# Fahien/rayca

Hardware: AMD Instinct MI355X
Metric: Mrays/sec (primary+shadow), 1920x1080 Sponza 1spp (higher is better)
Workload: dtype f32; 1 GPU; sponza-STAND-IN procedural atrium 271,568 tris, 1920x1080, primary + 1 shadow ray (Pathtracer max_depth=1, NEE, 1 point light), 1 spp; width=1920, height=1080, triangles=271568, bvh_nodes=135379, bvh_built_on=gpu (bvh_build.hip; same tree as the host builder), rays_per_frame=4146938, frames_in_flight=4, tiling=rows in bands of 8 dealt over 1 rank(s), frame_gather=none, launched_by=single process

## Files before the change

### __graft_entry__.py

```python
from __future__ import annotations

import os
import subprocess
import sys

ROOT = os.path.dirname(os.path.abspath(__file__))
CSRC = os.path.join(ROOT, "rayca_amd", "csrc")
LIB = os.path.join(CSRC, "librayca_hip.so")
HIPCC = os.environ.get("HIPCC", "/opt/rocm/bin/hipcc")
VARIANT_FLAGS = ["-DRAYCA_GEN_WAVES_PER_BLOCK=4", "-DRAYCA_COLD_ARGS=0"]
VARIANT_LIB = os.path.join(CSRC, "variants", "librayca_gen_earlier.so")

COMMON = ["-O3", "-std=c++17", "-fPIC", "-ffp-contract=off", "-fno-fast-math", "-Wall", "-Wno-unused-function",
          "-Wno-unused-result"]


def _stale(target, sources):
    if not os.path.exists(target):
        return True
    t = os.path.getmtime(target)
    return any(os.path.getmtime(s) > t for s in sources)


def build(force: bool = False) -> None:
    srcs = [os.path.join(CSRC, f) for f in ("kernels.hip", "refill.hip", "refill.hpp", "flavour.hpp", "trace_core.inc", "bvh_build.hip", "api.inc", "select.inc", "scene.inc", "multi.inc", "post.inc", "aux_kernels.inc", "general.inc", "wavefront.inc", "surface.inc", "image_pass.inc", "denoise.inc", "denoise_variance.inc", "temporal.inc", "upsample.inc", "tonemap.inc",
                                            "host_scene.cpp", "host_scene.hpp", "device_types.hpp", "no_pk.hpp", "rayca_math.hpp", "staging.hpp", "libm_exact.hpp")]
    srcs.append(os.path.join(ROOT, "include", "rayca_hip.h"))
    if force or _stale(LIB, srcs) or _stale(VARIANT_LIB, srcs):
        host_obj = os.path.join(CSRC, "host_scene.o")
        jobs = [subprocess.Popen(["g++", *COMMON, "-c", os.path.join(CSRC, "host_scene.cpp"), "-o", host_obj, "-pthread"])]
        objs = []
        for unit in ("kernels", "refill", "bvh_build"):
            obj = os.path.join(CSRC, unit + ".o")
            objs.append(obj)
            jobs.append(subprocess.Popen([HIPCC, "--offload-arch=gfx950", *COMMON, "-c", os.path.join(CSRC, unit + ".hip"), "-o", obj]))
        os.makedirs(os.path.dirname(VARIANT_LIB), exist_ok=True)
        variant_obj = os.path.join(os.path.dirname(VARIANT_LIB), "kernels_gen_earlier.o")
        jobs.append(subprocess.Popen([HIPCC, "--offload-arch=gfx950", *COMMON, *VARIANT_FLAGS, "-c", os.path.join(CSRC, "kernels.hip"), "-o", variant_obj]))
        failed = [j.args for j in jobs if j.wait() != 0]
        if failed:
            raise subprocess.CalledProcessError(1, failed[0])
        subprocess.run([HIPCC, "--offload-arch=gfx950", "-shared", "-fPIC", *objs, host_obj, "-o", LIB, "-lpthread"], check=True)
        subprocess.run([HIPCC, "--offload-arch=gfx950", "-shared", "-fPIC", variant_obj, *objs[1:], host_obj, "-o", VARIANT_LIB, "-lpthread"], check=True)
    subprocess.run(["make", "-s", "-C", os.path.join(ROOT, "oracle")], check=True)
    build_cpp_host()
    build_cpp_host("resident_draw")
    build_microbench()
    if ROOT not in sys.path:
        sys.path.insert(0, ROOT)
    import rayca_amd
    from rayca_amd import abi, lib
    l = lib.load()
    for sym in abi.PRODUCT_SYMBOLS:
        getattr(l, sym)


def build_microbench() -> None:
    out_dir = os.path.join(ROOT, "tests", "microbench", "_build")
    os.makedirs(out_dir, exist_ok=True)
    for name, extra, deps in (("peaks", [], []), ("libm_compare", ["-ffp-contract=off", "-fno-fast-math"], [os.path.join(CSRC, "libm_exact.hpp")])):
        src, exe = os.path.join(ROOT, "tests", "microbench", name + ".hip"), os.path.join(out_dir, name)
        if _stale(exe, [src] + deps):
            subprocess.run([HIPCC, "--offload-arch=gfx950", "-O3", "-std=c++17", *extra, src, "-o", exe], check=True)
# ... 55 lines not shown
```

### rayca_amd/csrc/api.inc

```
#include <dlfcn.h>

#include <algorithm>
#include <atomic>
#include <chrono>
#include <condition_variable>
#include <functional>
#include <memory>
#include <cstdio>
#include <cstdlib>
#include <cstring>
#include <mutex>
#include <string>
#include <thread>
#include <vector>

#include "refill.hpp"
#include "staging.hpp"

using namespace rayca;

namespace {

thread_local std::string g_last_error;

// ... 564 lines not shown
  return timed_launch(f.log, f.stream, refill ? RAYCA_KERNEL_SHADOW_REFILL : RAYCA_KERNEL_WF_SHADOW, f.timing, true, [&] {
    if (refill)
      launch_shadow_refill(gen0, sph, stats, lgrid, sp.lds_bytes, f.stream, *f.dscene, f.fp, q.in, q.in_count, sa, g, c->heads_b, c->counters, tl);
    else
      hipLaunchKernelGGL(kh, dim3(lgrid), dim3(kBlock), sp.lds_bytes, f.stream, *f.dscene, f.fp, q.in, q.in_count, wb, f.pb, g, c->counters, tl);
    return RAYCA_OK;
  });
}

GenChoice choose_generation(Frame& f, uint32_t g) {
  RaycaScene* s = f.s;
  const LaunchPlan& plan = f.plan;
  RaycaScene::Tune& tu = s->tune[plan.mode == kModePath ? 1 : 0][g == 0 ? 0 : 1];
  GenChoice ch{f.all_formats ? format_forced() : 0, false, false, false};
  const int refill_env = knobs().refill;
  const bool refill_possible = f.fused && plan.mode == kModeFlat && plan.ordered && s->dev.ref_leaf_of != nullptr;
  const int refill_forced = !refill_possible ? 0 : (f.opts.camera_rays == RAYCA_CAMERA_REFILL ? 1 : (f.opts.camera_rays == RAYCA_CAMERA_GENERATION ? 0 : refill_env));
  ch.refill = refill_forced > 0;
  bool kernel_pending = false;
  if (refill_possible && f.all_formats && refill_forced < 0) {
    std::lock_guard<std::mutex> tune_lock(s->tune_mu);
    if (tu.refill >= 0) ch.refill = tu.refill != 0;
    else if (f.pb.npix >= 65536u && !plan.stats && tu.refill_launched < 8u) {
      ch.refill = (tu.refill_launched++ & 1u) != 0;
      ch.refill_cal = true;
      if (ch.format < 0) ch.format = 1;
    } else {
      kernel_pending = true;
    }
  }
  const bool can_tune = plan.ordered && s->dev.ref_leaf_of != nullptr && wide_forced() < 0 && f.all_formats;
  if (can_tune && !ch.refill_cal && !kernel_pending) {
    const int cls = g == 0 ? 0 : 1;
    if (f.frame_format[cls] == -2) {
      std::lock_guard<std::mutex> tune_lock(s->tune_mu);
      f.frame_format[cls] = -1;
      if (tu.decided >= 0) f.frame_format[cls] = tu.decided;
      else if (f.pb.npix >= 65536u && !plan.stats && tu.launched < 16u) {
        f.frame_format[cls] = (int)(tu.launched++ & 3u);
        f.frame_calibrates[cls] = true;
      }
    }
    if (f.frame_format[cls] >= 0) ch.format = f.frame_format[cls];
    ch.calibrating = f.frame_calibrates[cls];
  }
  return ch;
}

int32_t fused_generation(Frame& f, uint32_t g, const GenQueues& q) {
  RaycaScene* s = f.s;
  FrameCtx* c = f.c;
  const GenChoice ch = choose_generation(f, g);
  const bool park = RAYCA_PARK_CTX && f.plan.mode == kModePath;
  const TravPlan tp = plan_traversal(s, f.plan.ordered, g, ch.format, park ? path_lds_entries() : kMaxLdsEntries);
  f.node_format |= (traits(tp.trav).wide ? (g == 0 ? 1u : 2u) : 0u) | (traits(tp.trav).half ? (g == 0 ? 4u : 8u) : 0u) | (ch.calibrating ? 256u : 0u) |
                   (ch.refill_cal ? 512u : 0u) | (ch.refill ? 1024u : 0u);
  const StackPlan sp = tp.stack;
  const uint32_t block = ch.refill ? (uint32_t)kBlock : (uint32_t)kGenBlock;
  const size_t lds_bytes = ((size_t)sp.lds_entries * 4u + (park ? (size_t)kCtxQuads * 16u : 0u)) * block;
  const bool sph = s->host.sphere_count != 0;
  GenKernel k = pick_kernel(f.plan.mode, g == 0, f.fused, tp.trav, sph, f.plan.stats);
  const RefillFlavour rf{tp.trav, sph, f.plan.stats};
  const uint32_t batches = g == 0 ? f.fp.tile_count : (f.pb.npix + 63u) / 64u;
  const uint32_t grid_mult = knobs().grid_mult;
  uint32_t grid = 0;
  TraceLaunch tl{};
  int32_t rc = persistent_grid(s, ch.refill ? flat_refill_kernel(rf) : reinterpret_cast<const void*>(k), lds_bytes, batches, true, f.in_flight, grid_mult, grid, block / 64u);
  if (rc != RAYCA_OK || (rc = bind_stack(c, sp, grid, tl, block)) != RAYCA_OK) return rc;
  const uint32_t ticket_forced = knobs().ticket;
  tl.ticket = ticket_forced ? ticket_forced : ticket_policy(batches, grid, block / 64u);
  size_t ev = 0;
  rc = timed_launch(f.log, f.stream, ch.refill ? RAYCA_KERNEL_FLAT_REFILL : RAYCA_KERNEL_GENERATION, f.timing || ch.calibrating || ch.refill_cal, true, [&] {
    if (ch.refill)
      launch_flat_refill(rf, grid, lds_bytes, f.stream, *f.dscene, f.fp, c->heads, f.rgba8, f.rgba32f, c->counters, tl);
    else
      hipLaunchKernelGGL(k, dim3(grid), dim3(kGenBlock), lds_bytes, f.stream,
                         GenArgs{*f.dscene, f.fp, c->heads, q.in, q.in_count, q.out, q.out_count, f.pb, g, f.rgba8, f.rgba32f, c->counters, tl});
    return RAYCA_OK;
  }, &ev);
  if (rc != RAYCA_OK) return rc;
  if (ch.calibrating) f.tune_events.push_back({g == 0 ? 0 : 1, ev, ch.format, -1});
  if (ch.refill_cal) f.tune_events.push_back({0, ev, ch.format, ch.refill ? 1 : 0});
  return RAYCA_OK;
}

int32_t stack_machine(Frame& f) {
  RaycaScene* s = f.s;
  FrameCtx* c = f.c;
  const RaycaConfig& cfg = f.cfg;
  GeneralKernel k = pick_general_kernel(s->dev.ref_leaf_of != nullptr, s->host.sphere_count != 0, f.plan.stats);
  const StackPlan sp = plan_stack(s->host.max_depth);
  uint32_t grid = 0;
  int32_t rc = persistent_grid(s, reinterpret_cast<const void*>(k), sp.lds_bytes, f.fp.tile_count, false, 1u, 0u, grid);
  if (rc != RAYCA_OK) return rc;
  uint32_t levels = 1;
  if (cfg.integrator == RAYCA_INTEGRATOR_PATHTRACER) levels = cfg.russian_roulette ? 64u : (cfg.max_depth ? cfg.max_depth : 1u);
  else if (cfg.integrator == RAYCA_INTEGRATOR_RAYTRACER || cfg.integrator == RAYCA_INTEGRATOR_SCRATCHER) levels = cfg.max_depth + 2u;
  if (levels > 256u) return fail(RAYCA_ERR_UNSUPPORTED, "max_depth too large for the path-vertex stack");
  GFrameStore store{};
  store.threads = grid * kBlock;
  store.levels = levels + 1u;
  if ((rc = grow_behind_pass(c, c->frames, (size_t)store.levels * 8u * store.threads * 16u)) != RAYCA_OK) return rc;
  store.frames = static_cast<float4*>(c->frames.ptr);
  if (cfg.direct_sampler == RAYCA_SAMPLER_MIS) {
    if ((rc = grow_behind_pass(c, c->mis_samples, (size_t)2u * kMisMaxSamples * store.threads * 16u)) != RAYCA_OK) return rc;
    store.samples = static_cast<float4*>(c->mis_samples.ptr);
  }
  TraceLaunch tl{};
  if ((rc = bind_stack(c, sp, grid, tl)) != RAYCA_OK) return rc;
  tl.ticket = f.fp.tile_count >= 16u * grid ? 2u : 1u;
  c->heads_clean = false;
  return timed_launch(f.log, f.stream, RAYCA_KERNEL_OTHER, f.timing, true, [&]() -> int32_t {
    HIP_TRY(hipMemsetAsync(c->heads, 0, 8 * kHeadStride * sizeof(uint32_t), f.stream));
// ... 771 lines not shown
```

### rayca_amd/csrc/kernels.hip

```cpp
#include "no_pk.hpp"
RAYCA_NO_PK_BEGIN
#include <hip/hip_runtime.h>
#include "device_types.hpp"
RAYCA_NO_PK_END

namespace rayca {
namespace {

RAYCA_NO_PK_BEGIN
#include "trace_core.inc"

#ifndef RAYCA_COLD_ARGS
#define RAYCA_COLD_ARGS 1
#endif
struct GenArgs {
  DevScene sc;
  FrameParams fp;
  uint32_t* heads;
  const QueuedRay* in_rays;
  const uint32_t* in_count;
  QueuedRay* out_rays;
  uint32_t* out_count;
  PathBuffers pb;
  uint32_t depth;
  uint8_t* rgba8;
  float4* rgba32f;
  TraceCounters* counters;
  TraceLaunch tl;
};
#if RAYCA_COLD_ARGS
#define GEN_COLD(member) cold_arg<decltype(GenArgs::member)>((uint32_t)offsetof(GenArgs, member))
#else
#define GEN_COLD(member) (a.member)
#endif
template <int MODE, bool GEN0, bool ORDERED, bool FUSED, bool FAST, bool SPH, bool WIDE, bool SPILL, bool STATS, bool HALF>
__global__ __launch_bounds__(kGenBlock, MODE == kModeFlat ? RAYCA_MIN_WAVES_FLAT : RAYCA_MIN_WAVES) void k_generation(GenArgs a) {
  const TraceLaunch& tl = a.tl;
  uint32_t* const heads = a.heads;
  const uint32_t depth = a.depth;
  extern __shared__ uint32_t lds_stack[];
  NodeStack<SPILL, kGenBlock> stack = make_stack<SPILL, kGenBlock>(lds_stack, tl, rc_bid() * kGenBlock + rc_tid());
  float4* const ctx_slot = reinterpret_cast<float4*>(lds_stack + tl.lds_entries * kGenBlock) + rc_tid();
  constexpr bool PARK = RAYCA_PARK_CTX && MODE == kModePath;
  const uint32_t lane = __lane_id();
  const uint32_t home = xcc_id();
  WorkCursor wc{};
  const uint32_t total = GEN0 ? GEN_COLD(fp).tile_count : (*GEN_COLD(in_count) + 63u) / 64u;
  LaneCounters cnt{};
  uint32_t n_shaded = 0, n_shadow = 0, n_bounce = 0;
  const bool collect_emissive = GEN0 ? true : (GEN_COLD(fp).direct_sampler == RAYCA_SAMPLER_NONE);
  const uint32_t nee_lights = (MODE == kModePath && GEN_COLD(fp).direct_sampler == RAYCA_SAMPLER_NEE) ? GEN_COLD(sc).light_count : 0u;

  for (;;) {
    const uint32_t batch = next_batch(heads, total, home, wc, tl.ticket);
    if (batch == RAYCA_NONE) break;
    bool live;
    uint32_t p = 0, key = 0;
    DRay ray;
    if (GEN0) {
      const FrameParams& fp = GEN_COLD(fp);
      const uint32_t ty = batch / fp.tiles_x, tx = batch - ty * fp.tiles_x;
      const uint32_t x = tx * kTileW + (lane & (kTileW - 1u)), r = ty * kTileH + (lane >> RAYCA_TILE_W_LOG2);
      live = x < fp.width && r < fp.rows;
      const uint32_t y = ((r / fp.band) * fp.parts + fp.part) * fp.band + (r % fp.band);
      p = r * fp.width + x;
      if (live) {
        ray = camera_ray(fp, x, y);
        key = rng_root(fp.seed, y * fp.width + x, fp.sample);
      }
    } else {
      const uint32_t i = batch * 64u + lane;
      live = i < *GEN_COLD(in_count);
      if (live) {
        const QueuedRay q = GEN_COLD(in_rays)[i];
        ray = make_ray(point3(q.ox, q.oy, q.oz), vec3(q.dx, q.dy, q.dz));
        p = q.pixel;
        key = q.key;
      }
    }
    const size_t slot = (size_t)depth * GEN_COLD(pb).npix + p;
    bool in_shadow = false;
    float t_stop = FLT_MAX;
    ShadeCtx cx;
    Color ns_x = black();
    Color direct = black();
    uint32_t li = 0, k = 0, dim = 0;
    const bool has_pixel = live;
    bool tail = false;

    while (live) {
      DHit hit;
      constexpr int kLeaveK = !ORDERED ? 0 : (MODE == kModeFlat ? RAYCA_LEAVE_K_CAMERA : (GEN0 ? RAYCA_LEAVE_K_PATH0 : RAYCA_LEAVE_K_BOUNCE));
      constexpr int kSlackForm = MODE == kModeFlat ? kSlackAlways : (GEN0 ? kSlackPerWave : kSlackNever);
      const bool found = trace<ORDERED, FAST, SPH, WIDE, SPILL, STATS, HALF, kLeaveK, kSlackForm>(a.sc, ray, t_stop, stack, hit, cnt);
      if (!in_shadow) {
        if (!found) {
          if (FUSED) direct = black() + black();
          else GEN_COLD(pb).state[slot] = kVertexNone;
          live = false;
        } else {
          n_shaded++;
          Color color;
          bool emissive;
          const PathBuffers& pb = GEN_COLD(pb);
          shade_hit<SPH>(GEN_COLD(sc), ray, hit, MODE == kModePath, color, emissive, cx);
          if (MODE == kModeFlat) {
            if (FUSED) direct = black() + color;
            else {
              pb.direct[slot] = as_f4(color);
              pb.state[slot] = kVertexEmissive;
            }
            live = false;
          } else if (collect_emissive && emissive) {
            pb.direct[slot] = as_f4(color);
            pb.state[slot] = kVertexEmissive;
            live = false;
          } else {
            in_shadow = true;
            if (PARK) {
              park_ctx<kGenBlock>(ctx_slot, cx);
              float zero = 0.0f;
              asm volatile("" : "+v"(zero));
              ctx_slot[6 * kGenBlock] = make_float4(zero, zero, zero, 1.0f);
            }
          }
        }
      } else {
        bool lit;
        if (t_stop == FLT_MAX) {
          lit = false;
          if (found) {
            const DevScene& sc = GEN_COLD(sc);
            const uint32_t hm = sc.ext[hit.prim].material;
            lit = hm != RAYCA_NONE && hm < sc.material_count && sc.materials[hm].emissive != 0u;
          }
        } else {
          lit = !(found && hit.t < t_stop);
        }
        if (PARK) {
          const Color sum = as_color(ctx_slot[6 * kGenBlock]) + (lit ? as_color(ctx_slot[5 * kGenBlock]) : black());
          ctx_slot[6 * kGenBlock] = as_f4(sum);
        } else {
          direct = direct + (lit ? ns_x : black());
        }
        if (++k == GEN_COLD(fp).light_samples) {
          k = 0;
          ++li;
        }
      }
      if (live && in_shadow) {
        bool pending = false;
        while (li < nee_lights) {
          if (PARK) cx = unpark_ctx<kGenBlock>(ctx_slot);
          const FrameParams& fp = GEN_COLD(fp);
          const NeeSample ns = nee_prepare(GEN_COLD(sc), fp, cx, li, k, key, dim, ray);
          const bool irrelevant = ORDERED && nee_irrelevant(ns);
          if (STATS) {
            const unsigned long long m = __ballot(irrelevant);
            if (m != 0ull && lane == (uint32_t)__ffsll((long long)m) - 1u) atomicAdd(&GEN_COLD(counters)->nee_irrelevant, (unsigned long long)__popcll(m));
          }
          if (irrelevant && fp.nee_skip) {
            if (++k == fp.light_samples) {
              k = 0;
              ++li;
            }
            continue;
          }
          if (PARK) ctx_slot[5 * kGenBlock] = as_f4(ns.x);
          else ns_x = ns.x;
          t_stop = ns.t_stop;
          pending = true;
          break;
        }
        if (!pending) {
          tail = true;
          live = false;
        }
      }
    }
    if (FUSED) {
      if (has_pixel) finalize_pixel(GEN_COLD(fp), direct, p, GEN_COLD(rgba8), GEN_COLD(rgba32f));
    } else if (MODE == kModePath) {
      const FrameParams& fp = GEN_COLD(fp);
      const PathBuffers& pb = GEN_COLD(pb);
      bool want_bounce = false;
      QueuedRay next{};
      if (tail) {
        const uint32_t limit = fp.direct_sampler != RAYCA_SAMPLER_NONE ? fp.max_depth - 1u : fp.max_depth;
        const bool hemi = fp.indirect_sampler == RAYCA_SAMPLER_HEMISPHERE;
        F4 sdir = vec3(0.0f, 0.0f, 0.0f);
        if (depth < limit) {
          const float e1 = rng_f32(key, dim++), e2 = rng_f32(key, dim++);
          const float theta = hemi ? rc_acosf(e1) : rc_acosf(sqrtf(e1));
          const float omega_a = 2.0f * kPi * e2;
          const float st = rc_sinf(theta);
          sdir = vec3(rc_cosf(omega_a) * st, rc_sinf(omega_a) * st, rc_cosf(theta));
        }
        if (PARK) {
          cx = unpark_ctx<kGenBlock>(ctx_slot);
          direct = as_color(ctx_slot[6 * kGenBlock]);
        }
        pb.direct[slot] = as_f4(direct);
        if (depth < limit) {
          const F4 w = cx.normal;
          const F4 a = close(w, vec3(0, 1, 0)) ? vec3(1, 0, 0) : vec3(0, 1, 0);
          const F4 u = normalized(cross(a, w));
          F4 v = cross(w, u);
          if (hemi) v = normalized(v);
          const F4 omega_i = (sdir.x * u + sdir.y * v) + sdir.z * w;
          const Color brdf = surf_brdf(cx, omega_i);
          Color factor;
          if (hemi) factor = ((2.0f * kPi) * brdf) * clampf(dot(cx.normal, omega_i), 0.0f, 1.0f);
          else factor = kPi * brdf;
          pb.brdf[slot] = as_f4(factor);
          pb.state[slot] = kVertexLit;
          if (depth + 1u < fp.max_depth) {
            want_bounce = true;
            next.ox = cx.next_origin.x; next.oy = cx.next_origin.y; next.oz = cx.next_origin.z;
            next.dx = omega_i.x; next.dy = omega_i.y; next.dz = omega_i.z;
            next.pixel = p;
            next.key = rng_child(key, 0u);
          }
        } else {
          pb.state[slot] = kVertexLitNoIndirect;
        }
      }
      n_shadow += (uint32_t)__popcll(__ballot(tail)) * nee_lights * fp.light_samples;
      n_bounce += (uint32_t)__popcll(__ballot(want_bounce));
      push_ray(want_bounce, next, GEN_COLD(out_rays), GEN_COLD(out_count));
    }
  }
  if (STATS) {
    unsigned long long b = cnt.boxes, t = cnt.tris, sh = n_shaded, sb = cnt.slot_boxes, stt = cnt.slot_tris;
    for (int off = 32; off > 0; off >>= 1) {
      b += __shfl_down(b, off);
      t += __shfl_down(t, off);
      sh += __shfl_down(sh, off);
      sb += __shfl_down(sb, off);
      stt += __shfl_down(stt, off);
    }
    if (lane == 0) {
      TraceCounters* const counters = GEN_COLD(counters);
      atomicAdd(&counters->boxes, b);
      atomicAdd(&counters->tris, t);
      atomicAdd(&counters->shaded, sh);
      atomicAdd(&counters->box_slots, sb);
      atomicAdd(&counters->tri_slots, stt);
    }
  }
  if (MODE == kModePath) {
    const unsigned long long s2 = n_shadow, b2 = n_bounce;
    if (lane == 0 && (s2 | b2)) {
      TraceCounters* const counters = GEN_COLD(counters);
// ... 125 lines not shown
```

### rayca_amd/csrc/select.inc

```
#ifndef RAYCA_WF_LDS_ENTRIES
#define RAYCA_WF_LDS_ENTRIES 16u
#endif

struct LaunchPlan {
  int mode;
  bool ordered, stats;
  bool wavefront;
  uint32_t generations;
};



using GenKernel = void (*)(GenArgs);
GenKernel pick_kernel(int mode, bool gen0, bool fused, Trav t, bool sph, bool stats) {
  const bool flat = mode == kModeFlat;
  return with_flavour([](auto T, auto FLAT, auto A, auto SPH, auto STATS) -> GenKernel {
    return k_generation<FLAT ? kModeFlat : kModePath, FLAT || A, T.ORDERED, FLAT && A, T.FAST, SPH, T.WIDE, T.SPILL, STATS, T.HALF>;
  }, t, flat, flat ? fused : gen0, sph, stats);
}

using TraceKernel = void (*)(DevScene, const float*, uint32_t, float*, uint32_t*, float*, TraceCounters*, TraceLaunch);
TraceKernel pick_trace_kernel(Trav t, bool sph, bool stats) {
  return with_flavour([](auto T, auto SPH, auto STATS) -> TraceKernel { return k_trace_rays<T.ORDERED, T.FAST, SPH, T.WIDE, T.SPILL, STATS>; }, t, sph, stats);
}
// ... 12 lines not shown
WfTraceKernel pick_wf_trace(bool gen0, Trav t, bool sph, bool stats) {
  return with_flavour([](auto T, auto GEN0, auto SPH, auto STATS) -> WfTraceKernel { return k_wf_trace<GEN0, T.FAST, SPH, T.SPILL, STATS>; }, t, gen0, sph, stats);
}
WfShadowKernel pick_wf_shadow(bool gen0, Trav t, bool sph, bool stats) {
  return with_flavour([](auto T, auto GEN0, auto SPH, auto STATS) -> WfShadowKernel { return k_wf_shadow<GEN0, T.FAST, SPH, T.SPILL, STATS>; }, t, gen0, sph, stats);
}
WfShadeKernel pick_wf_shade(int mode, bool gen0, bool fused, bool sph, bool rays) {
  const bool flat = mode == kModeFlat;
  return with_flags([](auto FLAT, auto A, auto SPH, auto RAYS) -> WfShadeKernel {
    return k_wf_shade<FLAT ? kModeFlat : kModePath, !RAYS && (FLAT || A), FLAT && (RAYS || A), SPH, RAYS>;
  }, flat, flat ? fused : gen0, sph, rays);
}

using GeneralKernel = void (*)(DevScene, FrameParams, uint32_t*, PathBuffers, GFrameStore, TraceCounters*, TraceLaunch);
GeneralKernel pick_general_kernel(bool fast, bool sph, bool stats) {
  return with_flags([](auto FAST, auto SPH, auto STATS) -> GeneralKernel { return k_general<true, FAST, SPH, true, STATS>; }, fast, sph, stats);
}

using SurfaceKernel = void (*)(DevScene, SurfaceIo);
SurfaceKernel pick_surface_kernel(bool sph) {
  return with_flags([](auto SPH) -> SurfaceKernel { return k_surface<SPH>; }, sph);
}

#ifndef RAYCA_MAX_LDS_ENTRIES
#define RAYCA_MAX_LDS_ENTRIES 24
#endif
constexpr uint32_t kMaxLdsEntries = RAYCA_MAX_LDS_ENTRIES;
struct StackPlan {
  uint32_t lds_entries, spill_entries;
  size_t lds_bytes;
};
StackPlan plan_stack(uint32_t need, uint32_t max_entries = kMaxLdsEntries) {
  StackPlan p;
  const uint32_t want = need + 1u;
  p.lds_entries = want < max_entries ? ((want + 3u) / 4u) * 4u : max_entries;
  if (p.lds_entries == 0) p.lds_entries = 4;
  p.spill_entries = want > p.lds_entries ? want - p.lds_entries : 0u;
  p.lds_bytes = (size_t)p.lds_entries * kBlock * 4u;
  return p;
}
int32_t bind_stack(FrameCtx* c, const StackPlan& sp, uint32_t grid, TraceLaunch& tl, uint32_t block_threads = kBlock) {
  tl = TraceLaunch{};
  tl.lds_entries = sp.lds_entries;
  if (sp.spill_entries) {
    tl.ovf_stride = grid * block_threads;
    const int32_t rc = grow_behind_pass(c, c->stack_spill, (size_t)sp.spill_entries * tl.ovf_stride * 4u);
    if (rc != RAYCA_OK) return rc;
    tl.ovf = static_cast<uint32_t*>(c->stack_spill.ptr);
  }
  return RAYCA_OK;
}

#ifndef RAYCA_PATH_LDS_ENTRIES
#define RAYCA_PATH_LDS_ENTRIES 12
#endif
struct Knobs {
  int format;
  int wavefront;
  bool wf_refill;
  int wf_shadow_refill;
  int refill;
  uint32_t grid_mult;
  uint32_t ticket;
  uint32_t path_lds_entries;
};
const Knobs& knobs() {
  static const Knobs k = [] {
    const auto env = [](const char* name, int unset) { const char* e = getenv(name); return e ? atoi(e) : unset; };
    Knobs n{};
    n.format = getenv("RAYCA_NODE_FORMAT") ? env("RAYCA_NODE_FORMAT", 0) & 3 : (getenv("RAYCA_WIDE") ? (env("RAYCA_WIDE", 0) ? 1 : 0) : -1);
    n.wavefront = env("RAYCA_WAVEFRONT", -1);
    n.wf_refill = env("RAYCA_WF_REFILL", 1) != 0;
    n.wf_shadow_refill = env("RAYCA_WF_SHADOW_REFILL", 1);
    n.refill = getenv("RAYCA_REFILL") ? (env("RAYCA_REFILL", 0) != 0 ? 1 : 0) : -1;
    n.grid_mult = (uint32_t)env("RAYCA_GRID_MULT", 0);
    n.ticket = (uint32_t)env("RAYCA_TICKET", 0);
    n.path_lds_entries = std::min(std::max((uint32_t)env("RAYCA_PATH_LDS_ENTRIES", RAYCA_PATH_LDS_ENTRIES), 4u), kMaxLdsEntries);
    return n;
  }();
  return k;
}

int format_forced() { return knobs().format; }
int wide_forced() {
  const int f = format_forced();
  return f < 0 ? -1 : (f & 1);
}
bool use_wide(uint32_t generation) {
  const int forced = wide_forced();
  return forced >= 0 ? forced != 0 : generation > 0;
}
uint32_t path_lds_entries() { return knobs().path_lds_entries; }

struct TreeFacts {
  bool fast;
  bool formats;
  bool half_nodes;
  uint32_t depth, depth4;
};
struct TravPlan {
  Trav trav;
  StackPlan stack;
};
TravPlan plan_traversal(const TreeFacts& tf, bool ordered, uint32_t generation, int format_choice, uint32_t max_lds_entries) {
  TravPlan tp{};
  const bool fast = tf.fast;
  const bool wide = ordered && fast && tf.formats && (format_choice >= 0 ? (format_choice & 1) != 0 : use_wide(generation));
  const bool half = ordered && fast && format_choice >= 0 && (format_choice & 2) != 0 && tf.formats && tf.half_nodes;
  tp.stack = plan_stack(wide ? tf.depth4 : tf.depth, max_lds_entries);
  if (!ordered) tp.trav = fast ? kTravFastAll : kTravExactAll;
  else if (!fast) tp.trav = kTravExact;
  else if (wide) tp.trav = half ? kTravFastWideHalf : kTravFastWide;
  else if (tp.stack.spill_entries) tp.trav = half ? kTravFastSpillHalf : kTravFastSpill;
  else tp.trav = half ? kTravFastHalf : kTravFast;
  return tp;
}
TravPlan plan_traversal(const RaycaScene* s, bool ordered, uint32_t generation, int format_choice = -1, uint32_t max_lds_entries = kMaxLdsEntries) {
  const bool formats = formats_ready(s);
  const TreeFacts tf{s->dev.ref_leaf_of != nullptr, formats, formats && s->dev_full.nodes_h != nullptr, s->host.max_depth, s->host.max_depth4};
  return plan_traversal(tf, ordered, generation, format_choice, max_lds_entries);
}

bool wavefront_by_default(uint32_t generations) {
  const int forced = knobs().wavefront;
  if (forced >= 0) return forced != 0;
  return generations >= 3u;
}

const char* generation_kernels_gap(const RaycaConfig& c) {
  if (c.integrator == RAYCA_INTEGRATOR_FLAT) return nullptr;
  if (c.integrator != RAYCA_INTEGRATOR_PATHTRACER) return "integrator";
  if (c.russian_roulette) return "russian_roulette";
  if (c.direct_sampler != RAYCA_SAMPLER_NONE && c.direct_sampler != RAYCA_SAMPLER_NEE) return "direct_sampler";
  const uint32_t limit = c.direct_sampler != RAYCA_SAMPLER_NONE ? (c.max_depth ? c.max_depth - 1u : 0u) : c.max_depth;
  const bool bounces = limit > 0 && c.max_depth > 0;
  if (bounces) {
    if (c.indirect_sampler != RAYCA_SAMPLER_COSINE && c.indirect_sampler != RAYCA_SAMPLER_HEMISPHERE) return "indirect_sampler";
    if (c.light_samples != 1) return "light_samples";
  }
  return nullptr;
}
bool nee_meets_directional_light(const RaycaScene* s, const RaycaConfig& c) {
  if (c.integrator == RAYCA_INTEGRATOR_PATHTRACER && c.direct_sampler == RAYCA_SAMPLER_NEE)
    for (const HostLight& l : s->host.lights)
      if (l.kind == RAYCA_LIGHT_DIRECTIONAL) return true;
// ... 25 lines not shown
    plan.mode = kModeGeneral;
    plan.generations = 1;
    return RAYCA_OK;
  }
  plan.mode = kModePath;
  plan.generations = c.max_depth;
  return RAYCA_OK;
}

int32_t kernel_registers(const void* k, uint32_t& regs) {
  static std::mutex mu;
  static std::vector<std::pair<const void*, uint32_t>> cache;
  std::lock_guard<std::mutex> lock(mu);
  for (const auto& e : cache)
    if (e.first == k) { regs = e.second; return RAYCA_OK; }
  hipFuncAttributes fa{};
  HIP_TRY(hipFuncGetAttributes(&fa, k));
  regs = fa.numRegs > 0 ? (uint32_t)fa.numRegs : 128u;
  cache.emplace_back(k, regs);
  return RAYCA_OK;
}

uint32_t grid_policy(uint32_t regs, size_t lds_bytes, uint32_t batches, bool capped, uint32_t in_flight, uint32_t per_cu_forced, uint32_t cu_count,
                     uint32_t block_waves) {
  const uint32_t blocks_per_unit = 4u / block_waves;
  uint32_t per_cu = per_cu_forced;
  if (per_cu == 0) {
    const size_t unit_lds = lds_bytes * blocks_per_unit;
    per_cu = std::min(512u / (((regs + 7u) / 8u) * 8u), unit_lds ? (uint32_t)((160u * 1024u) / unit_lds) : 8u);
    if (capped) {
      per_cu = std::max(1u, std::min(per_cu, 8u));
      if (in_flight >= 4u) per_cu = (per_cu + 1u) / 2u;
      else if (in_flight >= 2u) per_cu = (per_cu * 3u + 3u) / 4u;
    }
    per_cu = std::max(1u, per_cu);
  }
  const uint32_t need = (batches + block_waves - 1u) / block_waves;
  return std::min(cu_count * per_cu * blocks_per_unit, need ? need : 1u);
}
int32_t persistent_grid(const RaycaScene* s, const void* kernel, size_t lds_bytes, uint32_t batches, bool capped, uint32_t in_flight,
                        uint32_t per_cu_forced, uint32_t& grid, uint32_t block_waves = 4u) {
  uint32_t regs = 0;
  if (per_cu_forced == 0) {
    const int32_t rc = kernel_registers(kernel, regs);
    if (rc != RAYCA_OK) return rc;
  }
  grid = grid_policy(regs, lds_bytes, batches, capped, in_flight, per_cu_forced, (uint32_t)s->cu_count, block_waves);
  return RAYCA_OK;
}
uint32_t ticket_policy(uint32_t batches, uint32_t grid, uint32_t block_waves) { return batches >= 4u * block_waves * grid ? 2u : 1u; }

int32_t selftest_grid_policy(std::string& err) {
  struct Case { uint32_t regs; size_t wave_lds; uint32_t batches; bool capped; uint32_t in_flight, forced, waves; const char* what; };
  constexpr uint32_t kCus = 256u, kPathLds = 12u * 256u + 7u * 1024u;
  const Case cases[] = {
      {125u, kPathLds, 32400u, true, 4u, 0u, 2048u, "the 1080p path frame, four in flight: 8 waves per CU"},
      {125u, kPathLds, 32400u, true, 2u, 0u, 3072u, "the 1080p path frame, two in flight: 12 waves per CU"},
      {125u, kPathLds, 32400u, true, 1u, 0u, 4096u, "the 1080p path frame alone: 16 waves per CU"},
      {96u, 24u * 256u, 32400u, true, 1u, 0u, 5120u, "a Flat frame at 96 VGPRs: registers admit 5 waves per SIMD, LDS 6"},
      {64u, 0u, 32400u, false, 1u, 0u, 8192u, "no LDS, uncapped: 8 waves per SIMD"},
      {40u, 256u, 1u << 20, false, 1u, 0u, 12288u, "uncapped at 40 VGPRs and a little LDS: 12 waves per SIMD"},
      {40u, 256u, 1u << 20, true, 1u, 0u, 8192u, "the same, capped: 8"},
      {125u, kPathLds, 32400u, true, 4u, 3u, 3072u, "RAYCA_GRID_MULT=3 replaces the policy"},
      {256u, 96u * 1024u, 32400u, true, 4u, 0u, 1024u, "a kernel nothing admits still gets one wave per SIMD"},
  };
  const auto fail_case = [&](const std::string& what) { err = "grid_policy: " + what; return RAYCA_ERR_BAD_ARG; };
  for (const Case& c : cases)
    for (uint32_t w : {1u, 2u, 4u}) {
      const uint32_t grid = grid_policy(c.regs, c.wave_lds * w, c.batches, c.capped, c.in_flight, c.forced, kCus, w);
      if (grid * w != c.waves) return fail_case(std::string(c.what) + ": " + std::to_string(grid) + " workgroups of " + std::to_string(w) + " waves, expected " + std::to_string(c.waves) + " waves");
    }
  const uint32_t small[][4] = {{0u, 1u, 1u, 1u}, {1u, 1u, 1u, 1u}, {6u, 6u, 3u, 2u}, {42u, 42u, 21u, 11u}, {2047u, 2047u, 1024u, 512u}};
  for (const auto& r : small)
    for (uint32_t i = 0; i < 3u; ++i)
      if (const uint32_t grid = grid_policy(125u, kPathLds << i, r[0], true, 4u, 0u, kCus, 1u << i); grid != r[1 + i])
        return fail_case(std::to_string(r[0]) + " batches in workgroups of " + std::to_string(1u << i) + " waves: " + std::to_string(grid) + " workgroups, expected " + std::to_string(r[1 + i]));
  for (uint32_t regs : {24u, 64u, 96u, 125u, 128u, 200u})
    for (uint32_t wave_lds : {0u, 1024u, 6144u, 10240u, 16384u})
      for (uint32_t batches : {0u, 1u, 5u, 700u, 32400u, 129600u})
        for (uint32_t in_flight : {1u, 2u, 3u, 4u, 8u})
          for (int capped = 0; capped < 2; ++capped) {
            const uint32_t w4 = grid_policy(regs, (size_t)wave_lds * 4u, 1u << 30, capped != 0, in_flight, 0u, kCus, 4u) * 4u;
            for (uint32_t w : {1u, 2u, 4u}) {
              const uint32_t full = grid_policy(regs, (size_t)wave_lds * w, 1u << 30, capped != 0, in_flight, 0u, kCus, w);
              const uint32_t grid = grid_policy(regs, (size_t)wave_lds * w, batches, capped != 0, in_flight, 0u, kCus, w);
              const std::string tuple = "(" + std::to_string(regs) + " VGPRs, " + std::to_string(wave_lds) + " B per wave, " + std::to_string(batches) + " batches, " +
                                        std::to_string(in_flight) + " in flight, capped " + std::to_string(capped) + ", " + std::to_string(w) + " waves per workgroup)";
              if (full * w != w4 || w4 % (4u * kCus) != 0u) return fail_case(tuple + ": " + std::to_string(full * w) + " waves fill the chip, " + std::to_string(w4) + " in 256-thread blocks");
              if (grid == 0u || grid > full || (grid < full && grid != std::max(1u, (batches + w - 1u) / w))) return fail_case(tuple + ": " + std::to_string(grid) + " workgroups");
            }
          }
  const uint32_t tickets[][4] = {{32400u, 2048u, 1u, 2u}, {32400u, 512u, 4u, 2u}, {32400u, 4096u, 1u, 2u}, {8192u, 2048u, 1u, 2u}, {8191u, 2048u, 1u, 1u}, {8191u, 512u, 4u, 1u}, {6u, 6u, 1u, 1u}};
  for (const auto& t : tickets)
    if (ticket_policy(t[0], t[1], t[2]) != t[3])
      return fail_case("ticket_policy(" + std::to_string(t[0]) + " batches, " + std::to_string(t[1]) + " workgroups of " + std::to_string(t[2]) + " waves) is not " + std::to_string(t[3]));
  return RAYCA_OK;
}

struct GenChoice {
  int format;
  bool calibrating;
  bool refill;
  bool refill_cal;
};

struct PickerFamily {
  const char* picker;
  std::vector<Trav> travs;
  int bits;
  std::function<const void*(Trav, uint32_t)> pick;
  std::function<uint32_t(Trav, uint32_t)> id;
};
int32_t check_family(const PickerFamily& f, std::string& err) {
  struct Picked { const void* kernel; uint32_t id; std::string tuple; };
  std::vector<Picked> v;
  for (Trav t : f.travs)
    for (uint32_t i = 0; i < (1u << f.bits); ++i) v.push_back({f.pick(t, i), f.id(t, i), "trav " + std::to_string(t) + ", flags " + std::to_string(i)});
  for (size_t i = 0; i < v.size(); ++i) {
    if (!v[i].kernel) { err = std::string(f.picker) + ": (" + v[i].tuple + ") gets no kernel"; return RAYCA_ERR_BAD_ARG; }
    for (size_t j = 0; j < i; ++j)
      if ((v[i].kernel == v[j].kernel) != (v[i].id == v[j].id)) {
        err = std::string(f.picker) + ": (" + v[j].tuple + ") and (" + v[i].tuple + (v[i].id == v[j].id ? ") must be one kernel and are two" : ") must be two kernels and are one");
        return RAYCA_ERR_BAD_ARG;
      }
  }
  return RAYCA_OK;
}
int32_t selftest_kernel_selection(std::string& err) {
// ... 53 lines not shown
```

### rayca_amd/csrc/trace_core.inc

```
constexpr int kBlock = 256;
#ifndef RAYCA_GEN_WAVES_PER_BLOCK
#define RAYCA_GEN_WAVES_PER_BLOCK 1
#endif
constexpr int kGenWaves = RAYCA_GEN_WAVES_PER_BLOCK;
constexpr int kGenBlock = 64 * kGenWaves;
static_assert(kGenWaves == 1 || kGenWaves == 2 || kGenWaves == 4, "k_generation's workgroup: 1, 2 or 4 waves");
#ifndef RAYCA_TRACE_MIN_WAVES
#define RAYCA_TRACE_MIN_WAVES 1
#endif
#ifndef RAYCA_MIN_WAVES_FLAT
#define RAYCA_MIN_WAVES_FLAT 5
#endif
#ifndef RAYCA_MIN_WAVES
#define RAYCA_MIN_WAVES 4
#endif

__device__ __forceinline__ uint32_t rc_tid() { return __builtin_amdgcn_workitem_id_x(); }
__device__ __forceinline__ uint32_t rc_bid() { return __builtin_amdgcn_workgroup_id_x(); }
__device__ __forceinline__ uint32_t rc_bdim() { return __builtin_amdgcn_workgroup_size_x(); }
__device__ __forceinline__ uint32_t rc_gdim() { return __builtin_amdgcn_grid_size_x() / __builtin_amdgcn_workgroup_size_x(); }

template <class T>
__device__ __forceinline__ const T& cold_arg(uint32_t offset) {
  typedef __attribute__((address_space(4))) const char ConstByte;
  ConstByte* p = (ConstByte*)__builtin_amdgcn_kernarg_segment_ptr();
  asm volatile("" : "+s"(p));
  return *(const T*)(p + offset);
}

struct DRay {
  F4 o, d, rd;
};
struct DHit {
  float t;
  uint32_t prim;
  float u, v;
};

__device__ __forceinline__ DRay make_ray(F4 origin, F4 dir) {
  DRay r;
  r.rd = reciprocal(dir);
  origin.w = 1.0f;
  r.o = origin;
  r.d = dir;
  return r;
}

__device__ __forceinline__ bool slab(float ax, float ay, float az, float bx, float by, float bz, const DRay& r, float& tmin_out) {
  const float t1x = __fmaf_rn(ax - r.o.x, r.rd.x, 0.0f), t2x = __fmaf_rn(bx - r.o.x, r.rd.x, 0.0f);
  const float t1y = __fmaf_rn(ay - r.o.y, r.rd.y, 0.0f), t2y = __fmaf_rn(by - r.o.y, r.rd.y, 0.0f);
  const float t1z = __fmaf_rn(az - r.o.z, r.rd.z, 0.0f), t2z = __fmaf_rn(bz - r.o.z, r.rd.z, 0.0f);
  const float tmax = fminf(fminf(fmaxf(t1x, t2x), fmaxf(t1y, t2y)), fminf(fmaxf(t1z, t2z), FLT_MAX));
  const float tmin = fmaxf(fmaxf(fminf(t1x, t2x), fminf(t1y, t2y)), fmaxf(fminf(t1z, t2z), -FLT_MAX));
  tmin_out = tmin;
  return tmax >= tmin && tmax > 0.0f;
}

#ifndef RAYCA_RAY_SLACK
#define RAYCA_RAY_SLACK 1
#endif
struct FastRay {
  float mx, my, mz, cx, cy, cz;
#if RAYCA_RAY_SLACK
  float slack;
  bool fixed;
#endif
};
__device__ __forceinline__ bool fix_axis(float& m, float& c, float o, float centre, float inv_scale) {
// ... 574 lines not shown
    return Color{f[0] / 255.0f, f[1] / 255.0f, f[2] / 255.0f, f[3] / 255.0f};
  }
  if (t.color_type == RAYCA_COLOR_RGBA8) {
    const uint8_t* p = base + idx * 4;
    return Color{(float)p[0] / 255.0f, (float)p[1] / 255.0f, (float)p[2] / 255.0f, (float)p[3] / 255.0f};
  }
  const uint8_t* p = base + idx * 3;
  return Color{(float)p[0] / 255.0f, (float)p[1] / 255.0f, (float)p[2] / 255.0f, 255.0f / 255.0f};
}

__device__ __forceinline__ bool tex_valid(const DevScene& sc, uint32_t t) { return t != RAYCA_NONE && t < sc.texture_count; }

__device__ __forceinline__ Color pbr_color(const DevScene& sc, const DevMaterial& m, F2 uv) {
  const Color c = load_color(m.color);
  if (tex_valid(sc, m.albedo_texture)) return c * sample_texture(sc, m.albedo_texture, uv);
  return c;
}
__device__ __forceinline__ void pbr_metallic_roughness(const DevScene& sc, const DevMaterial& m, F2 uv, float& metallic, float& roughness) {
  if (tex_valid(sc, m.metallic_roughness_texture)) {
    const Color c = sample_texture(sc, m.metallic_roughness_texture, uv);
    metallic = c.b;
    roughness = c.r;
  } else {
    metallic = m.metallic_factor;
    roughness = m.roughness_factor;
  }
}
__device__ __forceinline__ DevMaterial default_material() {
  DevMaterial m{};
  m.color[0] = m.color[1] = m.color[2] = m.color[3] = 1.0f;
  m.ambient[3] = m.emission[3] = m.diffuse[3] = m.specular[3] = 1.0f;
  m.kind = RAYCA_MATERIAL_PBR;
  m.albedo_texture = m.normal_texture = m.metallic_roughness_texture = RAYCA_NONE;
  m.metallic_factor = 0.0f;
  m.roughness_factor = 1.0f;
  return m;
}

__device__ __forceinline__ F4 interp3(const float (*a)[3], float bu, float bv) {
  const float w2 = 1.0f - bu - bv;
  return (load_vec3(a[2]) * w2 + load_vec3(a[0]) * bu) + load_vec3(a[1]) * bv;
}

struct ShadeCtx {
  F4 point, normal, view, next_origin;
  Color kd, ks;
  float roughness, shininess;
  uint32_t kind;
};

#ifndef RAYCA_PARK_CTX
#define RAYCA_PARK_CTX 1
#endif
constexpr uint32_t kCtxQuads = 7;
template <int STRIDE = kBlock>
__device__ __forceinline__ void park_ctx(float4* slot, const ShadeCtx& c) {
  slot[0 * STRIDE] = make_float4(c.point.x, c.point.y, c.point.z, c.roughness);
  slot[1 * STRIDE] = make_float4(c.normal.x, c.normal.y, c.normal.z, c.shininess);
  slot[2 * STRIDE] = make_float4(c.view.x, c.view.y, c.view.z, __uint_as_float(c.kind));
  slot[3 * STRIDE] = make_float4(c.kd.r, c.kd.g, c.kd.b, c.kd.a);
  slot[4 * STRIDE] = make_float4(c.ks.r, c.ks.g, c.ks.b, c.ks.a);
}
template <int STRIDE = kBlock>
__device__ __forceinline__ ShadeCtx unpark_ctx(const float4* slot) {
  const float4 q0 = slot[0 * STRIDE], q1 = slot[1 * STRIDE], q2 = slot[2 * STRIDE], q3 = slot[3 * STRIDE], q4 = slot[4 * STRIDE];
  ShadeCtx c;
  c.point = f4(q0.x, q0.y, q0.z, 1.0f);
  c.normal = vec3(q1.x, q1.y, q1.z);
  c.view = vec3(q2.x, q2.y, q2.z);
  c.next_origin = c.point + c.normal * kRayBias;
  c.kd = Color{q3.x, q3.y, q3.z, q3.w};
  c.ks = Color{q4.x, q4.y, q4.z, q4.w};
  c.roughness = q0.w;
  c.shininess = q1.w;
  c.kind = __float_as_uint(q2.w);
  return c;
}

template <bool SPH>
__device__ __forceinline__ void shade_hit(const DevScene& sc, const DRay& ray, const DHit& hit, bool full, Color& color, bool& emissive,
                                          ShadeCtx& cx) {
  const PrimExt& e = sc.ext[hit.prim];
  const float bu = hit.u, bv = hit.v;
  const float w2 = 1.0f - bu - bv;
  const bool is_sphere = SPH && e.kind == RAYCA_GEOMETRY_SPHERE;
  const Color geom_color = is_sphere ? white() : (load_color(e.color[2]) * w2 + load_color(e.color[0]) * bu) + load_color(e.color[1]) * bv;
  const F2 uv = is_sphere ? F2{0.0f, 0.0f}
                          : F2{(e.uv[2][0] * w2 + e.uv[0][0] * bu) + e.uv[1][0] * bv, (e.uv[2][1] * w2 + e.uv[0][1] * bu) + e.uv[1][1] * bv};
  const DevMaterial m = (e.material != RAYCA_NONE && e.material < sc.material_count) ? sc.materials[e.material] : default_material();
  Color mc;
  if (m.kind == RAYCA_MATERIAL_PBR) mc = pbr_color(sc, m, uv);
  else if (m.kind == RAYCA_MATERIAL_PHONG) mc = load_color(m.ambient) + load_color(m.emission);
  else mc = load_color(m.diffuse);
  color = geom_color * mc;
  emissive = m.emissive != 0u;
  if (!full) return;
  F4 normal;
  F4 point = ray.o + ray.d * hit.t;
  F4 hit_dir = ray.d;
  if (is_sphere) {
    const DevSphere& sp = sc.spheres[e.node];
    const DRay l = sphere_local_ray(sp, ray);
    hit_dir = l.d;
    const F4 model_point = l.o + l.d * hit.t;
    const Trs wt{f4(sp.translation[0], sp.translation[1], sp.translation[2], 0.0f), f4(sp.rotation[0], sp.rotation[1], sp.rotation[2], sp.rotation[3]),
                 f4(sp.scale[0], sp.scale[1], sp.scale[2], 0.0f)};
    point = trs_apply_point(wt, model_point);
    const F4 hp = mat4_apply_point(reinterpret_cast<const float(*)[4]>(sp.inv_mat4), point);
    const F4 mn = normalized(as_vec(hp - f4(sp.center[0], sp.center[1], sp.center[2], sp.center[3])));
    const float* nm = sp.normal_mat;
    float out[3] = {0.0f, 0.0f, 0.0f};
    const float in[3] = {mn.x, mn.y, mn.z};
    for (int i = 0; i < 3; ++i)
      for (int j = 0; j < 3; ++j) out[i] += nm[4 * i + j] * in[j];
    normal = normalized(vec3(out[0], out[1], out[2]));
  } else {
    normal = normalized(interp3(e.normal, bu, bv));
  }
  if (!is_sphere && m.kind == RAYCA_MATERIAL_PBR && tex_valid(sc, m.normal_texture)) {
    const F4 tangent = normalized(interp3(e.tangent, bu, bv));
    const F4 bitangent = normalized(interp3(e.bitangent, bu, bv));
    F4 sn = premultiplied(sample_texture(sc, m.normal_texture, uv));
    sn = sn * 2.0f - f4(1.0f, 1.0f, 1.0f, 1.0f);
    normal = normalized(mat3_apply(mat3_tbn(tangent, bitangent, normal), sn));
  }
  cx.normal = normal;
  cx.point = point;
  cx.view = -hit_dir;
  cx.next_origin = cx.point + normal * kRayBias;
// ... 238 lines not shown
```

Measured before the change: 15450 Mrays/s.

## Compact parked shading context in LDS and raise path kernel occupancy to five waves

Shrinks the per-thread LDS context park from seven quads to five quads plus six words. It does this by merging roughness and shininess into one slot, keying off the material kind, and storing the premultiplied sample and its sum as scalars. With the smaller footprint, the path LDS stack drops to 4 entries, and launch bounds target 5 waves per SIMD for non-stats, non-sphere path kernels. The aim is more resident waves to hide traversal latency. The cost is fewer LDS stack rows (more spills to memory), tighter register budgets, and a possible change to rounding in the premultiplied sum.

```diff
diff --git a/__graft_entry__.py b/__graft_entry__.py
--- a/__graft_entry__.py
+++ b/__graft_entry__.py
@@ -8,7 +8,7 @@
 CSRC = os.path.join(ROOT, "rayca_amd", "csrc")
 LIB = os.path.join(CSRC, "librayca_hip.so")
 HIPCC = os.environ.get("HIPCC", "/opt/rocm/bin/hipcc")
-VARIANT_FLAGS = ["-DRAYCA_GEN_WAVES_PER_BLOCK=4", "-DRAYCA_COLD_ARGS=0"]
+VARIANT_FLAGS = ["-DRAYCA_GEN_WAVES_PER_BLOCK=4", "-DRAYCA_COLD_ARGS=0", "-DRAYCA_MIN_WAVES=4", "-DRAYCA_CTX_COMPACT=0"]
 VARIANT_LIB = os.path.join(CSRC, "variants", "librayca_gen_earlier.so")
 
 COMMON = ["-O3", "-std=c++17", "-fPIC", "-ffp-contract=off", "-fno-fast-math", "-Wall", "-Wno-unused-function",
diff --git a/rayca_amd/csrc/api.inc b/rayca_amd/csrc/api.inc
--- a/rayca_amd/csrc/api.inc
+++ b/rayca_amd/csrc/api.inc
@@ -640,13 +640,13 @@
   FrameCtx* c = f.c;
   const GenChoice ch = choose_generation(f, g);
   const bool park = RAYCA_PARK_CTX && f.plan.mode == kModePath;
-  const TravPlan tp = plan_traversal(s, f.plan.ordered, g, ch.format, park ? path_lds_entries() : kMaxLdsEntries);
+  const bool sph = s->host.sphere_count != 0;
+  const TravPlan tp = plan_traversal(s, f.plan.ordered, g, ch.format, park ? path_lds_entries(path_waves(f.plan.stats, sph)) : kMaxLdsEntries);
   f.node_format |= (traits(tp.trav).wide ? (g == 0 ? 1u : 2u) : 0u) | (traits(tp.trav).half ? (g == 0 ? 4u : 8u) : 0u) | (ch.calibrating ? 256u : 0u) |
                    (ch.refill_cal ? 512u : 0u) | (ch.refill ? 1024u : 0u);
   const StackPlan sp = tp.stack;
   const uint32_t block = ch.refill ? (uint32_t)kBlock : (uint32_t)kGenBlock;
-  const size_t lds_bytes = ((size_t)sp.lds_entries * 4u + (park ? (size_t)kCtxQuads * 16u : 0u)) * block;
-  const bool sph = s->host.sphere_count != 0;
+  const size_t lds_bytes = ((size_t)sp.lds_entries * 4u + (park ? (size_t)kCtxBytes : 0u)) * block;
   GenKernel k = pick_kernel(f.plan.mode, g == 0, f.fused, tp.trav, sph, f.plan.stats);
   const RefillFlavour rf{tp.trav, sph, f.plan.stats};
   const uint32_t batches = g == 0 ? f.fp.tile_count : (f.pb.npix + 63u) / 64u;
diff --git a/rayca_amd/csrc/kernels.hip b/rayca_amd/csrc/kernels.hip
--- a/rayca_amd/csrc/kernels.hip
+++ b/rayca_amd/csrc/kernels.hip
@@ -34,13 +34,13 @@
 #define GEN_COLD(member) (a.member)
 #endif
 template <int MODE, bool GEN0, bool ORDERED, bool FUSED, bool FAST, bool SPH, bool WIDE, bool SPILL, bool STATS, bool HALF>
-__global__ __launch_bounds__(kGenBlock, MODE == kModeFlat ? RAYCA_MIN_WAVES_FLAT : RAYCA_MIN_WAVES) void k_generation(GenArgs a) {
+__global__ __launch_bounds__(kGenBlock, MODE == kModeFlat ? RAYCA_MIN_WAVES_FLAT : path_waves(STATS, SPH)) void k_generation(GenArgs a) {
   const TraceLaunch& tl = a.tl;
   uint32_t* const heads = a.heads;
   const uint32_t depth = a.depth;
   extern __shared__ uint32_t lds_stack[];
   NodeStack<SPILL, kGenBlock> stack = make_stack<SPILL, kGenBlock>(lds_stack, tl, rc_bid() * kGenBlock + rc_tid());
-  float4* const ctx_slot = reinterpret_cast<float4*>(lds_stack + tl.lds_entries * kGenBlock) + rc_tid();
+  const CtxSlot ctx_slot{lds_stack + tl.lds_entries * kGenBlock};
   constexpr bool PARK = RAYCA_PARK_CTX && MODE == kModePath;
   const uint32_t lane = __lane_id();
   const uint32_t home = xcc_id();
@@ -119,9 +119,7 @@
             in_shadow = true;
             if (PARK) {
               park_ctx<kGenBlock>(ctx_slot, cx);
-              float zero = 0.0f;
-              asm volatile("" : "+v"(zero));
-              ctx_slot[6 * kGenBlock] = make_float4(zero, zero, zero, 1.0f);
+              park_sum_reset<kGenBlock>(ctx_slot);
             }
           }
         }
@@ -138,8 +136,7 @@
           lit = !(found && hit.t < t_stop);
         }
         if (PARK) {
-          const Color sum = as_color(ctx_slot[6 * kGenBlock]) + (lit ? as_color(ctx_slot[5 * kGenBlock]) : black());
-          ctx_slot[6 * kGenBlock] = as_f4(sum);
+          park_sum_add<kGenBlock>(ctx_slot, lit);
         } else {
           direct = direct + (lit ? ns_x : black());
         }
@@ -166,7 +163,7 @@
             }
             continue;
           }
-          if (PARK) ctx_slot[5 * kGenBlock] = as_f4(ns.x);
+          if (PARK) park_sample<kGenBlock>(ctx_slot, ns.x);
           else ns_x = ns.x;
           t_stop = ns.t_stop;
           pending = true;
@@ -198,7 +195,7 @@
         }
         if (PARK) {
           cx = unpark_ctx<kGenBlock>(ctx_slot);
-          direct = as_color(ctx_slot[6 * kGenBlock]);
+          direct = unpark_sum<kGenBlock>(ctx_slot);
         }
         pb.direct[slot] = as_f4(direct);
         if (depth < limit) {
diff --git a/rayca_amd/csrc/select.inc b/rayca_amd/csrc/select.inc
--- a/rayca_amd/csrc/select.inc
+++ b/rayca_amd/csrc/select.inc
@@ -88,7 +88,10 @@
 }
 
 #ifndef RAYCA_PATH_LDS_ENTRIES
-#define RAYCA_PATH_LDS_ENTRIES 12
+#define RAYCA_PATH_LDS_ENTRIES (RAYCA_CTX_COMPACT ? 4 : 12)
+#endif
+#ifndef RAYCA_PATH_LDS_ENTRIES_FOUR_WAVES
+#define RAYCA_PATH_LDS_ENTRIES_FOUR_WAVES 12
 #endif
 struct Knobs {
   int format;
@@ -111,7 +114,7 @@
     n.refill = getenv("RAYCA_REFILL") ? (env("RAYCA_REFILL", 0) != 0 ? 1 : 0) : -1;
     n.grid_mult = (uint32_t)env("RAYCA_GRID_MULT", 0);
     n.ticket = (uint32_t)env("RAYCA_TICKET", 0);
-    n.path_lds_entries = std::min(std::max((uint32_t)env("RAYCA_PATH_LDS_ENTRIES", RAYCA_PATH_LDS_ENTRIES), 4u), kMaxLdsEntries);
+    n.path_lds_entries = getenv("RAYCA_PATH_LDS_ENTRIES") ? std::min(std::max((uint32_t)env("RAYCA_PATH_LDS_ENTRIES", 0), 4u), kMaxLdsEntries) : 0u;
     return n;
   }();
   return k;
@@ -126,7 +129,10 @@
   const int forced = wide_forced();
   return forced >= 0 ? forced != 0 : generation > 0;
 }
-uint32_t path_lds_entries() { return knobs().path_lds_entries; }
+uint32_t path_lds_entries(int waves_per_simd) {
+  if (const uint32_t forced = knobs().path_lds_entries) return forced;
+  return std::min(std::max((uint32_t)(waves_per_simd >= 5 ? RAYCA_PATH_LDS_ENTRIES : RAYCA_PATH_LDS_ENTRIES_FOUR_WAVES), 4u), kMaxLdsEntries);
+}
 
 struct TreeFacts {
   bool fast;
@@ -258,16 +264,20 @@
 
 int32_t selftest_grid_policy(std::string& err) {
   struct Case { uint32_t regs; size_t wave_lds; uint32_t batches; bool capped; uint32_t in_flight, forced, waves; const char* what; };
-  constexpr uint32_t kCus = 256u, kPathLds = 12u * 256u + 7u * 1024u;
+  constexpr uint32_t kCus = 256u, kPathLds = 4u * 256u + 104u * 64u;
   const Case cases[] = {
-      {125u, kPathLds, 32400u, true, 4u, 0u, 2048u, "the 1080p path frame, four in flight: 8 waves per CU"},
-      {125u, kPathLds, 32400u, true, 2u, 0u, 3072u, "the 1080p path frame, two in flight: 12 waves per CU"},
-      {125u, kPathLds, 32400u, true, 1u, 0u, 4096u, "the 1080p path frame alone: 16 waves per CU"},
+      {96u, kPathLds, 32400u, true, 4u, 0u, 3072u, "the 1080p path frame, four in flight: 12 waves per CU"},
+      {96u, kPathLds, 32400u, true, 2u, 0u, 4096u, "the 1080p path frame, two in flight: 16 waves per CU"},
+      {96u, kPathLds, 32400u, true, 1u, 0u, 5120u, "the 1080p path frame alone: 20 waves per CU, by its 96 registers and by its LDS"},
+      {64u, kPathLds, 32400u, false, 1u, 0u, 5120u, "its LDS alone admits 20 waves per CU (21 in single waves: counted in units of four)"},
+      {120u, 12u * 256u + 104u * 64u, 32400u, true, 1u, 0u, 4096u, "a counting or sphere path frame, four waves per SIMD and twelve rows, 9 728 B: 16 waves per CU"},
+      {112u, 12u * 256u + 7u * 1024u, 32400u, true, 4u, 0u, 2048u, "the path frame with seven quads, twelve rows and 112 registers, four in flight: 8 waves per CU"},
+      {112u, 12u * 256u + 7u * 1024u, 32400u, true, 1u, 0u, 4096u, "the same alone: 16 waves per CU"},
       {96u, 24u * 256u, 32400u, true, 1u, 0u, 5120u, "a Flat frame at 96 VGPRs: registers admit 5 waves per SIMD, LDS 6"},
       {64u, 0u, 32400u, false, 1u, 0u, 8192u, "no LDS, uncapped: 8 waves per SIMD"},
       {40u, 256u, 1u << 20, false, 1u, 0u, 12288u, "uncapped at 40 VGPRs and a little LDS: 12 waves per SIMD"},
       {40u, 256u, 1u << 20, true, 1u, 0u, 8192u, "the same, capped: 8"},
-      {125u, kPathLds, 32400u, true, 4u, 3u, 3072u, "RAYCA_GRID_MULT=3 replaces the policy"},
+      {96u, kPathLds, 32400u, true, 4u, 2u, 2048u, "RAYCA_GRID_MULT=2 replaces the policy"},
       {256u, 96u * 1024u, 32400u, true, 4u, 0u, 1024u, "a kernel nothing admits still gets one wave per SIMD"},
   };
   const auto fail_case = [&](const std::string& what) { err = "grid_policy: " + what; return RAYCA_ERR_BAD_ARG; };
@@ -279,7 +289,7 @@
   const uint32_t small[][4] = {{0u, 1u, 1u, 1u}, {1u, 1u, 1u, 1u}, {6u, 6u, 3u, 2u}, {42u, 42u, 21u, 11u}, {2047u, 2047u, 1024u, 512u}};
   for (const auto& r : small)
     for (uint32_t i = 0; i < 3u; ++i)
-      if (const uint32_t grid = grid_policy(125u, kPathLds << i, r[0], true, 4u, 0u, kCus, 1u << i); grid != r[1 + i])
+      if (const uint32_t grid = grid_policy(96u, kPathLds << i, r[0], true, 4u, 0u, kCus, 1u << i); grid != r[1 + i])
         return fail_case(std::to_string(r[0]) + " batches in workgroups of " + std::to_string(1u << i) + " waves: " + std::to_string(grid) + " workgroups, expected " + std::to_string(r[1 + i]));
   for (uint32_t regs : {24u, 64u, 96u, 125u, 128u, 200u})
     for (uint32_t wave_lds : {0u, 1024u, 6144u, 10240u, 16384u})
diff --git a/rayca_amd/csrc/trace_core.inc b/rayca_amd/csrc/trace_core.inc
--- a/rayca_amd/csrc/trace_core.inc
+++ b/rayca_amd/csrc/trace_core.inc
@@ -12,8 +12,9 @@
 #define RAYCA_MIN_WAVES_FLAT 5
 #endif
 #ifndef RAYCA_MIN_WAVES
-#define RAYCA_MIN_WAVES 4
-#endif
+#define RAYCA_MIN_WAVES 5
+#endif
+constexpr int path_waves(bool stats, bool sph) { return stats || sph ? 4 : RAYCA_MIN_WAVES; }
 
 __device__ __forceinline__ uint32_t rc_tid() { return __builtin_amdgcn_workitem_id_x(); }
 __device__ __forceinline__ uint32_t rc_bid() { return __builtin_amdgcn_workgroup_id_x(); }
@@ -694,17 +695,47 @@
 #ifndef RAYCA_PARK_CTX
 #define RAYCA_PARK_CTX 1
 #endif
-constexpr uint32_t kCtxQuads = 7;
+#ifndef RAYCA_CTX_COMPACT
+#define RAYCA_CTX_COMPACT 1
+#endif
+#if RAYCA_CTX_COMPACT
+constexpr uint32_t kCtxQuads = 5, kCtxWords = 6;
+#else
+constexpr uint32_t kCtxQuads = 7, kCtxWords = 0;
+#endif
+constexpr uint32_t kCtxBytes = kCtxQuads * 16u + kCtxWords * 4u;
+struct CtxSlot {
+  uint32_t* base;
+};
+template <int STRIDE>
+__device__ __forceinline__ uint32_t ctx_tid() {
+  if (STRIDE != 64) return rc_tid();
+  uint32_t l;
+  asm volatile("v_mbcnt_lo_u32_b32 %0, -1, 0\n\tv_mbcnt_hi_u32_b32 %0, -1, %0" : "=v"(l));
+  return l;
+}
+template <int STRIDE>
+__device__ __forceinline__ float4* ctx_quads(const CtxSlot& s) { return reinterpret_cast<float4*>(s.base) + ctx_tid<STRIDE>(); }
+template <int STRIDE>
+__device__ __forceinline__ float* ctx_words(const CtxSlot& s) { return reinterpret_cast<float*>(s.base + kCtxQuads * 4u * STRIDE) + ctx_tid<STRIDE>(); }
 template <int STRIDE = kBlock>
-__device__ __forceinline__ void park_ctx(float4* slot, const ShadeCtx& c) {
+__device__ __forceinline__ void park_ctx(const CtxSlot& s, const ShadeCtx& c) {
+  float4* const slot = ctx_quads<STRIDE>(s);
+#if RAYCA_CTX_COMPACT
+  slot[0 * STRIDE] = make_float4(c.point.x, c.point.y, c.point.z, c.kind == RAYCA_MATERIAL_PHONG ? c.shininess : c.roughness);
+  slot[1 * STRIDE] = make_float4(c.normal.x, c.normal.y, c.normal.z, __uint_as_float(c.kind));
+  slot[2 * STRIDE] = make_float4(c.view.x, c.view.y, c.view.z, 0.0f);
+#else
   slot[0 * STRIDE] = make_float4(c.point.x, c.point.y, c.point.z, c.roughness);
   slot[1 * STRIDE] = make_float4(c.normal.x, c.normal.y, c.normal.z, c.shininess);
   slot[2 * STRIDE] = make_float4(c.view.x, c.view.y, c.view.z, __uint_as_float(c.kind));
+#endif
   slot[3 * STRIDE] = make_float4(c.kd.r, c.kd.g, c.kd.b, c.kd.a);
   slot[4 * STRIDE] = make_float4(c.ks.r, c.ks.g, c.ks.b, c.ks.a);
 }
 template <int STRIDE = kBlock>
-__device__ __forceinline__ ShadeCtx unpark_ctx(const float4* slot) {
+__device__ __forceinline__ ShadeCtx unpark_ctx(const CtxSlot& s) {
+  const float4* const slot = ctx_quads<STRIDE>(s);
   const float4 q0 = slot[0 * STRIDE], q1 = slot[1 * STRIDE], q2 = slot[2 * STRIDE], q3 = slot[3 * STRIDE], q4 = slot[4 * STRIDE];
   ShadeCtx c;
   c.point = f4(q0.x, q0.y, q0.z, 1.0f);
@@ -713,10 +744,68 @@
   c.next_origin = c.point + c.normal * kRayBias;
   c.kd = Color{q3.x, q3.y, q3.z, q3.w};
   c.ks = Color{q4.x, q4.y, q4.z, q4.w};
+#if RAYCA_CTX_COMPACT
+  c.roughness = c.shininess = q0.w;
+  c.kind = __float_as_uint(q1.w);
+#else
   c.roughness = q0.w;
   c.shininess = q1.w;
   c.kind = __float_as_uint(q2.w);
+#endif
   return c;
+}
+template <int STRIDE = kBlock>
+__device__ __forceinline__ void park_sum_reset(const CtxSlot& s) {
+  float zero = 0.0f;
+  asm volatile("" : "+v"(zero));
+#if RAYCA_CTX_COMPACT
+  float* const words = ctx_words<STRIDE>(s);
+  words[3 * STRIDE] = zero;
+  words[4 * STRIDE] = zero;
+  words[5 * STRIDE] = zero;
+#else
+  ctx_quads<STRIDE>(s)[6 * STRIDE] = make_float4(zero, zero, zero, 1.0f);
+#endif
+}
+template <int STRIDE = kBlock>
+__device__ __forceinline__ void park_sample(const CtxSlot& s, Color x) {
+#if RAYCA_CTX_COMPACT
+  float* const words = ctx_words<STRIDE>(s);
+  words[0 * STRIDE] = x.r * x.a;
+  words[1 * STRIDE] = x.g * x.a;
+  words[2 * STRIDE] = x.b * x.a;
+#else
+  ctx_quads<STRIDE>(s)[5 * STRIDE] = make_float4(x.r, x.g, x.b, x.a);
+#endif
+}
+template <int STRIDE = kBlock>
+__device__ __forceinline__ void park_sum_add(const CtxSlot& s, bool lit) {
+#if RAYCA_CTX_COMPACT
+  float* const words = ctx_words<STRIDE>(s);
+  const float r = words[3 * STRIDE] + (lit ? words[0 * STRIDE] : 0.0f);
+  const float g = words[4 * STRIDE] + (lit ? words[1 * STRIDE] : 0.0f);
+  const float b = words[5 * STRIDE] + (lit ? words[2 * STRIDE] : 0.0f);
+  words[3 * STRIDE] = r;
+  words[4 * STRIDE] = g;
+  words[5 * STRIDE] = b;
+#else
+  float4* const quads = ctx_quads<STRIDE>(s);
+  const float4 a = quads[6 * STRIDE], x = quads[5 * STRIDE];
+  const Color sum = Color{a.x, a.y, a.z, a.w} + (lit ? Color{x.x, x.y, x.z, x.w} : black());
+  quads[6 * STRIDE] = make_float4(sum.r, sum.g, sum.b, sum.a);
+#endif
+}
+template <int STRIDE = kBlock>
+__device__ __forceinline__ Color unpark_sum(const CtxSlot& s) {
+#if RAYCA_CTX_COMPACT
+  const float* const words = ctx_words<STRIDE>(s);
+  float one = 1.0f;
+  asm volatile("" : "+v"(one));
+  return Color{words[3 * STRIDE], words[4 * STRIDE], words[5 * STRIDE], one};
+#else
+  const float4 a = ctx_quads<STRIDE>(s)[6 * STRIDE];
+  return Color{a.x, a.y, a.z, a.w};
+#endif
 }
 
 template <bool SPH>
```

Measured after the change: 16540 Mrays/s (median of 6 runs). +7.1%, better.
